# silence-tang/GaussianIP

Measured on AMD Instinct MI355X. Metric: raster_fwd_bwd_mpix_per_s, higher is better.
Workload: dtype f32

## Files before the change

gaussianip_amd/csrc/api.hip:

```cpp
#include <string.h>

#include "gip_internal.h"

static inline size_t align256(size_t x) { return (x + 255) & ~(size_t)255; }

static_assert(offsetof(GipRasterConfig, antialiasing) == 188 && sizeof(GipRasterConfig) == 192, "GipRasterConfig layout");

static bool sh_mfma_path(const GipRasterConfig* c) { return c->sh_coeffs > 0 && c->sh_degree >= 1 && c->V >= 2 && !c->sh_scalar; }

static bool valid_config(const GipRasterConfig* c) {
  if (!c) return false;
  if (c->P < 0 || c->V < 1 || c->V > GIP_MAX_VIEWS || c->H < 1 || c->W < 1) return false;
  if (c->sh_degree < 0 || c->sh_degree > 3) return false;
  if (c->capacity < 1 || c->capacity > 0xfffffff0ull) return false;
  if ((c->H + GIP_TILE - 1) / GIP_TILE > 0xffff || (c->W + GIP_TILE - 1) / GIP_TILE > 0xffff) return false;
  return true;
}

extern "C" int gip_abi_version(void) { return GIP_ABI_VERSION; }

extern "C" const char* gip_status_string(int status) {
  switch (status) {
    case GIP_OK: return "ok";
    case GIP_ERR_BAD_ARGUMENT: return "bad argument (null pointer, or not exactly one of shs/colors_precomp and scales+rotations/cov3D_precomp)";
    case GIP_ERR_BUFFER_TOO_SMALL: return "state or scratch buffer smaller than gip_raster_state_bytes()/gip_raster_scratch_bytes()";
    case GIP_ERR_HIP: return "HIP runtime error";
    case GIP_ERR_UNSUPPORTED: return "unsupported configuration";
    default: return "unknown status";
  }
}

extern "C" int gip_raster_state_layout(const GipRasterConfig* c, GipRasterStateLayout* L) {
  if (!valid_config(c) || !L) return GIP_ERR_BAD_ARGUMENT;
  memset(L, 0, sizeof(*L));
  const size_t P = (size_t)c->P, V = (size_t)c->V;
  L->tiles_x = (uint32_t)((c->W + GIP_TILE - 1) / GIP_TILE);
  L->tiles_y = (uint32_t)((c->H + GIP_TILE - 1) / GIP_TILE);
  L->num_blocks = (uint32_t)((c->P + GIP_BLOCK - 1) / GIP_BLOCK);
  const size_t T = (size_t)L->tiles_x * L->tiles_y, nblk = L->num_blocks;
  size_t off = 0;
  L->header = off;       off = align256(off + sizeof(GipRasterHeader));
  L->tile_count = off;   off = align256(off + V * T * 4);
  L->tile_cursor = off;  off = align256(off + V * T * 4);
  L->tile_count_b = off; off = align256(off + V * T * 4);
  L->tile_start = off;   off = align256(off + (V * T + 1) * 4);
  L->block_sums = off;   off = align256(off + (V * nblk + 1) * 4);
  L->block_offset = off; off = align256(off + (V * nblk + 1) * 4);
  L->records = off;      off = align256(off + V * P * GIP_RECORD_BYTES);
  L->inst_offset = off;  off = align256(off + V * P * 4);
  L->inst_slot = off;    off = align256(off + V * P * GIP_SLOTS * 4);
  L->n_contrib = off;    off = align256(off + V * (size_t)c->H * c->W * 4);
  L->final_T = off;      off = align256(off + V * (size_t)c->H * c->W * 4);
  L->tile_order = off;   off = align256(off + V * T * 4);
  const size_t ckpt_cap = (size_t)c->capacity / GIP_SEGMENT + 1, seg_cap = ckpt_cap + V * T;
  L->seg_start = off;    off = align256(off + (V * T + 1) * 4);
  L->ckpt_start = off;   off = align256(off + (V * T + 1) * 4);
  L->seg_tile = off;     off = align256(off + seg_cap * 4);
  L->checkpoints = off;  off = align256(off + ckpt_cap * GIP_CKPT_FLOATS * 256 * sizeof(float));
  L->keys = off;         off = align256(off + (size_t)c->capacity * 8);
  L->sh_colors = off;    off = align256(off + (sh_mfma_path(c) ? V * P * 4 * sizeof(float) : 0));
  L->total = off;
  return GIP_OK;
}

extern "C" size_t gip_raster_state_bytes(const GipRasterConfig* c) {
  GipRasterStateLayout L;
  if (gip_raster_state_layout(c, &L) != GIP_OK) return 0;
  return L.total;
}

extern "C" size_t gip_raster_scratch_bytes(const GipRasterConfig* c) {
  if (!valid_config(c)) return 0;
  return align256((size_t)c->capacity * GIP_PARTIAL_FLOATS * sizeof(float));
}

static void fill_params(const GipRasterConfig* c, const GipRasterStateLayout& L, GipKernelParams* kp) {
  memset(kp, 0, sizeof(*kp));
  kp->P = c->P; kp->V = c->V; kp->H = c->H; kp->W = c->W;
  kp->tiles_x = (int)L.tiles_x; kp->tiles_y = (int)L.tiles_y; kp->T = kp->tiles_x * kp->tiles_y;
  kp->nblk = (int)L.num_blocks;
  kp->D = c->sh_degree; kp->M = c->sh_coeffs;
  kp->scale_modifier = c->scale_modifier;
  kp->capacity = (uint32_t)c->capacity;
  kp->exact_lists = c->exact_lists ? 1 : 0;
  kp->forward_only = c->forward_only ? 1 : 0;
  kp->sh_mfma = sh_mfma_path(c) ? 1 : 0;
  kp->antialiasing = c->antialiasing ? 1 : 0;
  kp->ckpt_capacity = (uint32_t)(c->capacity / GIP_SEGMENT + 1);
  kp->seg_capacity = kp->ckpt_capacity + (uint32_t)(kp->V * kp->T);
  for (int v = 0; v < c->V; v++) {
    kp->view[v].tanfovx = c->tanfovx[v];
    kp->view[v].tanfovy = c->tanfovy[v];
    kp->view[v].focal_x = c->W / (2.0f * c->tanfovx[v]);
    kp->view[v].focal_y = c->H / (2.0f * c->tanfovy[v]);
  }
}

static GipStatePtrs state_ptrs(void* state, const GipRasterStateLayout& L) {
  char* b = (char*)state;
  GipStatePtrs p;
  p.header = (GipRasterHeader*)(b + L.header);
  p.records = (GipRecord*)(b + L.records);
  p.inst_offset = (uint32_t*)(b + L.inst_offset);
  p.tile_count = (uint32_t*)(b + L.tile_count);
  p.tile_start = (uint32_t*)(b + L.tile_start);
  p.tile_cursor = (uint32_t*)(b + L.tile_cursor);
  p.tile_count_b = (uint32_t*)(b + L.tile_count_b);
  p.inst_slot = (uint32_t*)(b + L.inst_slot);
  p.block_sums = (uint32_t*)(b + L.block_sums);
  p.block_offset = (uint32_t*)(b + L.block_offset);
  p.keys = (unsigned long long*)(b + L.keys);
  p.n_contrib = (uint32_t*)(b + L.n_contrib);
  p.final_T = (float*)(b + L.final_T);
  p.tile_order = (uint32_t*)(b + L.tile_order);
  p.seg_start = (uint32_t*)(b + L.seg_start);
  p.ckpt_start = (uint32_t*)(b + L.ckpt_start);
  p.seg_tile = (uint32_t*)(b + L.seg_tile);
  p.checkpoints = (float*)(b + L.checkpoints);
  p.sh_colors = (float*)(b + L.sh_colors);
  p.host_header = nullptr;
  return p;
}

// ... 42 lines not shown
        float ms = 0.f;
        if (hipEventElapsedTime(&ms, ev[2 * i], ev[2 * i + 1]) != hipSuccess) rc = GIP_ERR_HIP;
        out[i] = ms;
      }
    }
    for (int i = 0; i < created; i++) (void)hipEventDestroy(ev[i]);
    return rc;
  }
};
}

static int forward_impl(const GipRasterConfig* cfg, const GipRasterInputs* in, const GipRasterOutputs* out,
                        void* state, size_t state_bytes, void* stream, float* times) {
  if (!valid_config(cfg)) return cfg && (cfg->V > GIP_MAX_VIEWS || cfg->sh_degree > 3) ? GIP_ERR_UNSUPPORTED : GIP_ERR_BAD_ARGUMENT;
  int rc = check_inputs(cfg, in);
  if (rc != GIP_OK) return rc;
  if (!out || !out->color || !out->radii || !out->depth || !out->alpha || !state) return GIP_ERR_BAD_ARGUMENT;
  GipRasterStateLayout L;
  gip_raster_state_layout(cfg, &L);
  if (state_bytes < L.total) return GIP_ERR_BUFFER_TOO_SMALL;
  GipKernelParams kp;
  fill_params(cfg, L, &kp);
  if (!in->shs) kp.sh_mfma = 0;
  GipStatePtrs st = state_ptrs(state, L);
  st.host_header = out->host_header;
  hipStream_t s = (hipStream_t)stream;
  StageTimer tm(s, times);

  tm.begin(GIP_STAGE_CLEAR);
  HIP_TRY(hipMemsetAsync((char*)state + L.header, 0, L.tile_start - L.header, s));
  tm.end(GIP_STAGE_CLEAR);
  if (cfg->P > 0) {
    tm.begin(GIP_STAGE_PREPROCESS);
    if (kp.sh_mfma) gip_launch_sh_forward_mfma(kp, *in, st.sh_colors, s);
    gip_launch_preprocess(kp, *in, out->radii, st, s);
    tm.end(GIP_STAGE_PREPROCESS);
    LAUNCH_CHECK();
  }
  tm.begin(GIP_STAGE_SCAN);
  gip_launch_scan(kp, st, s);
  tm.end(GIP_STAGE_SCAN);
  LAUNCH_CHECK();
  if (cfg->P > 0) {
    tm.begin(GIP_STAGE_SCATTER);
    gip_launch_scatter(kp, st, s);
    tm.end(GIP_STAGE_SCATTER);
    LAUNCH_CHECK();
// ... 14 lines not shown
  return forward_impl(cfg, in, out, state, state_bytes, stream, nullptr);
}
extern "C" int gip_raster_forward_profiled(const GipRasterConfig* cfg, const GipRasterInputs* in, const GipRasterOutputs* out,
                                           void* state, size_t state_bytes, void* stream, float* times_ms) {
  if (!times_ms) return GIP_ERR_BAD_ARGUMENT;
  return forward_impl(cfg, in, out, state, state_bytes, stream, times_ms);
}

static int backward_impl(const GipRasterConfig* cfg, const GipRasterInputs* in, const GipRasterGradsIn* gin,
                         const void* state, size_t state_bytes, void* scratch, size_t scratch_bytes,
                         const GipRasterGradsOut* gout, void* stream, float* times) {
  if (!valid_config(cfg)) return GIP_ERR_BAD_ARGUMENT;
  int rc = check_inputs(cfg, in);
  if (rc != GIP_OK) return rc;
  if (!gin || !gin->alpha || !gin->color || !gin->depth || !gout || !state || !scratch) return GIP_ERR_BAD_ARGUMENT;
  if (cfg->forward_only) return GIP_ERR_BAD_ARGUMENT;
  GipRasterStateLayout L;
  gip_raster_state_layout(cfg, &L);
  if (state_bytes < L.total || scratch_bytes < gip_raster_scratch_bytes(cfg)) return GIP_ERR_BUFFER_TOO_SMALL;
  if (cfg->P == 0) return GIP_OK;
  GipKernelParams kp;
  fill_params(cfg, L, &kp);
  if (!in->shs) kp.sh_mfma = 0;
  GipStatePtrs st = state_ptrs(const_cast<void*>(state), L);
  hipStream_t s = (hipStream_t)stream;
  StageTimer tm(s, times);
  tm.begin(GIP_STAGE_RENDER_BWD);
  gip_launch_render_backward(kp, in->bg, st, *gin, (float*)scratch, s);
  tm.end(GIP_STAGE_RENDER_BWD);
  LAUNCH_CHECK();
  tm.begin(GIP_STAGE_GATHER_BWD);
  gip_launch_gather_backward(kp, *in, st, (const float*)scratch, *gout, s);
  if (kp.sh_mfma && (gout->dL_dshs || gout->dL_dmeans3D)) gip_launch_sh_backward_mfma(kp, *in, st, st.sh_colors, *gout, s);
  tm.end(GIP_STAGE_GATHER_BWD);
  LAUNCH_CHECK();
  return tm.finish();
}

extern "C" int gip_raster_backward(const GipRasterConfig* cfg, const GipRasterInputs* in, const GipRasterGradsIn* gin,
                                   const void* state, size_t state_bytes, void* scratch, size_t scratch_bytes,
                                   const GipRasterGradsOut* gout, void* stream) {
  return backward_impl(cfg, in, gin, state, state_bytes, scratch, scratch_bytes, gout, stream, nullptr);
}
extern "C" int gip_raster_backward_profiled(const GipRasterConfig* cfg, const GipRasterInputs* in, const GipRasterGradsIn* gin,
                                            const void* state, size_t state_bytes, void* scratch, size_t scratch_bytes,
                                            const GipRasterGradsOut* gout, void* stream, float* times_ms) {
  if (!times_ms) return GIP_ERR_BAD_ARGUMENT;
// ... 18 lines not shown
```

gaussianip_amd/csrc/binning.hip:

```cpp
#include "gip_internal.h"

#define SCAN_THREADS 1024
#define SCAN_WAVES (SCAN_THREADS / 64)
#define SCAN_CHUNK SCAN_THREADS

__device__ __forceinline__ uint32_t nseg_of(uint32_t count) { return (count + GIP_SEGMENT - 1) / GIP_SEGMENT; }

#define ORDER_CLASSES 6
__device__ __forceinline__ int class_of(uint32_t c) {
  return c >= 2048 ? 0 : c >= 1024 ? 1 : c >= 512 ? 2 : c >= 128 ? 3 : c >= 1 ? 4 : 5;
}

__device__ __forceinline__ uint32_t block_excl_scan(uint32_t v, uint32_t* s_w, uint32_t* total) {
  const int lane = threadIdx.x & 63, wave = threadIdx.x >> 6;
  const uint32_t incl = gip_wave_incl_scan_u32(v);
  __syncthreads();
  if (lane == 63) s_w[wave] = incl;
  __syncthreads();
  uint32_t base = 0, tot = 0;
#pragma unroll
  for (int w = 0; w < SCAN_WAVES; w++) { const uint32_t x = s_w[w]; base += w < wave ? x : 0u; tot += x; }
  *total = tot;
  return base + incl - v;
}

__device__ __forceinline__ uint32_t wave_sum_u32(uint32_t v) {
#pragma unroll
  for (int d = 32; d >= 1; d >>= 1) v += (uint32_t)__shfl_xor((int)v, d, 64);
  return v;
}

__global__ void __launch_bounds__(SCAN_THREADS)
gip_scan_kernel(GipKernelParams kp, const uint32_t* __restrict__ tile_count, const uint32_t* __restrict__ tile_count_b,
                uint32_t* __restrict__ tile_start,
                uint32_t* __restrict__ seg_start, uint32_t* __restrict__ ckpt_start,
                const uint32_t* __restrict__ block_sums, uint32_t* __restrict__ block_offset,
                uint32_t* __restrict__ tile_order, GipRasterHeader* __restrict__ header, uint32_t* __restrict__ host_header) {
  __shared__ uint32_t s_w[SCAN_WAVES];
  __shared__ uint32_t s_acc[2][3 + ORDER_CLASSES];
  __shared__ uint32_t s_max;
  __shared__ uint32_t s_cls[ORDER_CLASSES][SCAN_WAVES];
  const int n = kp.V * kp.T;
  const int n_chunks = (n + SCAN_CHUNK - 1) / SCAN_CHUNK;
  const int tid = threadIdx.x, lane = tid & 63, wave = tid >> 6;
  if ((int)blockIdx.x >= n_chunks) {
    const int nb = kp.V * kp.nblk;
    const int c0 = ((int)blockIdx.x - n_chunks) * SCAN_CHUNK;
    uint32_t before = 0;
    for (int i0 = tid; i0 < c0; i0 += 8 * SCAN_THREADS) {
      uint32_t v8[8];
#pragma unroll
      for (int u = 0; u < 8; u++) { const int i = i0 + u * SCAN_THREADS; v8[u] = i < c0 ? block_sums[i] : 0u; }
#pragma unroll
      for (int u = 0; u < 8; u++) before += v8[u];
    }
    before = wave_sum_u32(before);
    if (tid == 0) s_max = 0u;
    __syncthreads();
    if (lane == 0) atomicAdd(&s_max, before);
    __syncthreads();
    const uint32_t base = s_max;
    const int i = c0 + tid;
    const uint32_t v = i < nb ? block_sums[i] : 0u;
    uint32_t total;
    const uint32_t e = block_excl_scan(v, s_w, &total);
    if (i < nb) block_offset[i] = base + e;
    if (c0 + SCAN_CHUNK >= nb && tid == 0) block_offset[nb] = base + total;
    return;
  }
  const int chunk0 = (int)blockIdx.x * SCAN_CHUNK;
  if (tid < 2 * (3 + ORDER_CLASSES)) (&s_acc[0][0])[tid] = 0u;
  if (tid == 0) s_max = 0u;
  __syncthreads();
  uint32_t b_c = 0, b_s = 0, b_k = 0, t_c = 0, t_s = 0, t_k = 0, mx = 0;
  uint32_t b_cls[ORDER_CLASSES], t_cls[ORDER_CLASSES];
#pragma unroll
  for (int c = 0; c < ORDER_CLASSES; c++) { b_cls[c] = 0; t_cls[c] = 0; }
  for (int i0 = wave * 64; i0 < n; i0 += 8 * SCAN_THREADS) {
    uint32_t va[8], vb[8];
#pragma unroll
    for (int u = 0; u < 8; u++) {
      const int i = i0 + u * SCAN_THREADS + lane;
      va[u] = i < n ? tile_count[i] : 0u;
      vb[u] = i < n ? tile_count_b[i] : 0u;
    }
#pragma unroll
    for (int u = 0; u < 8; u++) {
      const int g0 = i0 + u * SCAN_THREADS;
      if (g0 >= n) break;
      const int i = g0 + lane;
      const uint32_t c = va[u] + vb[u], a = nseg_of(c), k = a ? a - 1 : 0;
      const int cls = i < n ? class_of(c) : -1;
      const bool before = g0 < chunk0;
      t_c += c; t_s += a; t_k += k;
      mx = c > mx ? c : mx;
      if (before) { b_c += c; b_s += a; b_k += k; }
#pragma unroll
      for (int q = 0; q < ORDER_CLASSES; q++) {
        const uint32_t m = (uint32_t)__popcll(__ballot(cls == q));
        t_cls[q] += m;
        if (before) b_cls[q] += m;
      }
    }
  }
  b_c = wave_sum_u32(b_c); b_s = wave_sum_u32(b_s); b_k = wave_sum_u32(b_k);
  t_c = wave_sum_u32(t_c); t_s = wave_sum_u32(t_s); t_k = wave_sum_u32(t_k);
  mx = gip_wave_max_u32(mx);
  if (lane == 0) {
    atomicAdd(&s_acc[0][0], b_c); atomicAdd(&s_acc[0][1], b_s); atomicAdd(&s_acc[0][2], b_k);
    atomicAdd(&s_acc[1][0], t_c); atomicAdd(&s_acc[1][1], t_s); atomicAdd(&s_acc[1][2], t_k);
#pragma unroll
    for (int q = 0; q < ORDER_CLASSES; q++) { atomicAdd(&s_acc[0][3 + q], b_cls[q]); atomicAdd(&s_acc[1][3 + q], t_cls[q]); }
    atomicMax(&s_max, mx);
  }
  __syncthreads();
  const int i = chunk0 + tid;
  uint32_t c = 0;
  if (i < n) c = tile_count[i] + tile_count_b[i];
  const uint32_t a = nseg_of(c), k = a ? a - 1 : 0;
  uint32_t tot;
  const uint32_t e_c = block_excl_scan(c, s_w, &tot);
  const uint32_t e_s = block_excl_scan(a, s_w, &tot);
  const uint32_t e_k = block_excl_scan(k, s_w, &tot);
  if (i < n) {
    tile_start[i] = s_acc[0][0] + e_c;
    seg_start[i] = s_acc[0][1] + e_s;
    ckpt_start[i] = s_acc[0][2] + e_k;
  }
  const int cls = i < n ? class_of(c) : -1;
  uint32_t rank = 0;
#pragma unroll
  for (int q = 0; q < ORDER_CLASSES; q++) {
    const unsigned long long m = __ballot(cls == q);
    if (cls == q) rank = (uint32_t)__popcll(m & ((1ull << lane) - 1ull));
    if (lane == 0) s_cls[q][wave] = (uint32_t)__popcll(m);
  }
  __syncthreads();
  if (cls >= 0) {
    uint32_t pos = rank + s_acc[0][3 + cls];
#pragma unroll
    for (int q = 0; q < ORDER_CLASSES; q++) pos += q < cls ? s_acc[1][3 + q] : 0u;
    for (int w = 0; w < wave; w++) pos += s_cls[cls][w];
    tile_order[pos] = (uint32_t)i;
  }
  if (blockIdx.x == 0 && tid == 0) {
    const uint32_t total = s_acc[1][0];
    tile_start[n] = total; seg_start[n] = s_acc[1][1]; ckpt_start[n] = s_acc[1][2];
    const uint32_t n0 = s_acc[1][3], n1 = s_acc[1][4], n2 = s_acc[1][5], n3 = s_acc[1][6], n4 = s_acc[1][7];
    header->class_end[1] = n0;
    header->class_end[2] = n0 + n1;
    header->class_end[0] = n0 + n1 + n2;
    header->class_end[3] = n0 + n1 + n2 + n3 + n4;
    header->abi_version = GIP_ABI_VERSION;
    header->num_rendered = total;
    header->overflow = (total > kp.capacity) ? 1u : 0u;
    header->max_tile_count = s_max;
    header->num_segments = s_acc[1][1];
    header->num_checkpoints = s_acc[1][2];
    if (host_header) {
      host_header[0] = GIP_ABI_VERSION; host_header[1] = total;
      host_header[2] = (total > kp.capacity) ? 1u : 0u; host_header[3] = s_max;
    }
  }
}

void gip_launch_scan(const GipKernelParams& kp, GipStatePtrs st, hipStream_t s) {
  const int n = kp.V * kp.T, nb = kp.V * kp.nblk;
  const int n_chunks = (n + SCAN_CHUNK - 1) / SCAN_CHUNK, b_chunks = nb > 0 ? (nb + SCAN_CHUNK - 1) / SCAN_CHUNK : 1;
  hipLaunchKernelGGL(gip_scan_kernel, dim3(n_chunks + b_chunks), dim3(SCAN_THREADS), 0, s, kp, st.tile_count, st.tile_count_b, st.tile_start,
                     st.seg_start, st.ckpt_start, st.block_sums, st.block_offset, st.tile_order, st.header, st.host_header);
}

__global__ void __launch_bounds__(GIP_BLOCK)
gip_scatter_kernel(GipKernelParams kp, const GipRecord* __restrict__ records, const uint32_t* __restrict__ tile_start,
                   const uint32_t* __restrict__ tile_count, uint32_t* __restrict__ tile_cursor,
                   const uint32_t* __restrict__ inst_slot, const uint32_t* __restrict__ block_offset,
                   uint32_t* __restrict__ inst_offset, unsigned long long* __restrict__ keys) {
  const int v = blockIdx.y;
  const int idx = blockIdx.x * GIP_BLOCK + threadIdx.x;
  uint32_t tiles = 0, rmin = 0, rmax = 0, dbits = 0, tmask = 0;
  if (idx < kp.P) {
    const uint4* rp = reinterpret_cast<const uint4*>(records + (size_t)v * kp.P + idx);
    const uint4 q0 = rp[0], q1 = rp[1], q3 = rp[3];
    dbits = q0.z; tiles = q1.w; rmin = q3.x; rmax = q3.y; tmask = q3.w;
  }
  __shared__ uint32_t s_wave[4];
  const int lane = threadIdx.x & 63, wave = threadIdx.x >> 6;
  uint32_t incl = gip_wave_incl_scan_u32(tiles);
  if (lane == 63) s_wave[wave] = incl;
  __syncthreads();
  uint32_t base = block_offset[(size_t)v * kp.nblk + blockIdx.x];
  for (int w = 0; w < wave; w++) base += s_wave[w];
  if (idx < kp.P) inst_offset[(size_t)v * kp.P + idx] = base + incl - tiles;
// ... 389 lines not shown
```

gaussianip_amd/csrc/gip_internal.h:

```cpp
#pragma once
#include <hip/hip_runtime.h>
#include <stdint.h>

#include "../../include/gip_raster.h"

#define GIP_BLOCK 256
#define GIP_WAVE 64
#define GIP_NEAR 0.2f
#define GIP_ALPHA_MIN (1.0f / 255.0f)
#define GIP_ALPHA_MAX 0.99f
#define GIP_T_MIN 0.0001f

struct __attribute__((aligned(16))) GipRecord {
  float x, y, depth, opacity;
  float ca, cb, cc; uint32_t tiles;
  float r, g, b; int32_t radius;
  uint32_t rmin, rmax, clamped, tmask;
};

#define GIP_MASK_TILES 32
__host__ __device__ inline bool gip_rect_has(uint32_t tmask, int area, int k) { return area > GIP_MASK_TILES || ((tmask >> k) & 1u); }
__host__ __device__ inline int gip_rect_rank(uint32_t tmask, int area, int k) {
  return area > GIP_MASK_TILES ? k : __builtin_popcount(tmask & ((1u << k) - 1u));
}

static_assert(sizeof(GipRecord) == GIP_RECORD_BYTES, "record size");

struct GipViewConst {
  float tanfovx, tanfovy, focal_x, focal_y;
};

struct GipKernelParams {
  int P, V, H, W;
  int tiles_x, tiles_y, T;
  int nblk;
  int D, M;
  float scale_modifier;
  uint32_t capacity;
  uint32_t seg_capacity;
  uint32_t ckpt_capacity;
  int exact_lists;
  int forward_only;
  int sh_mfma;
  int antialiasing;
  GipViewConst view[GIP_MAX_VIEWS];
};

struct GipStatePtrs {
  GipRasterHeader* header;
  GipRecord* records;
  uint32_t* inst_offset;
  uint32_t* tile_count;
  uint32_t* tile_start;
  uint32_t* tile_cursor;
  uint32_t* tile_count_b;
  uint32_t* inst_slot;
  uint32_t* block_sums;
  uint32_t* block_offset;
  unsigned long long* keys;
  uint32_t* n_contrib;
  float* final_T;
  uint32_t* tile_order;
  uint32_t* seg_start;
  uint32_t* ckpt_start;
  uint32_t* seg_tile;
  float* checkpoints;
  uint32_t* host_header;
  float* sh_colors;
};

void gip_launch_preprocess(const GipKernelParams& kp, const GipRasterInputs& in, int32_t* radii, GipStatePtrs st, hipStream_t s);
void gip_launch_scan(const GipKernelParams& kp, GipStatePtrs st, hipStream_t s);
void gip_launch_scatter(const GipKernelParams& kp, GipStatePtrs st, hipStream_t s);
void gip_launch_tile_sort(const GipKernelParams& kp, GipStatePtrs st, hipStream_t s);
void gip_launch_render_forward(const GipKernelParams& kp, const float* bg, GipStatePtrs st, float* color, float* depth, float* alpha, hipStream_t s);
void gip_launch_render_backward(const GipKernelParams& kp, const float* bg, GipStatePtrs st, const GipRasterGradsIn& gin, float* partial, hipStream_t s);
void gip_launch_gather_backward(const GipKernelParams& kp, const GipRasterInputs& in, GipStatePtrs st, const float* partial, const GipRasterGradsOut& gout, hipStream_t s);
void gip_launch_sh_forward_mfma(const GipKernelParams& kp, const GipRasterInputs& in, float* sh_colors, hipStream_t s);
void gip_launch_sh_backward_mfma(const GipKernelParams& kp, const GipRasterInputs& in, GipStatePtrs st, const float* sh_gcol, const GipRasterGradsOut& gout, hipStream_t s);
void gip_launch_mark_visible(int P, const float* means3D, const float* view, uint8_t* present, hipStream_t s);

#ifdef __HIPCC__
__device__ __forceinline__ uint32_t gip_wave_incl_scan_u32(uint32_t v) {
  const int lane = threadIdx.x & 63;
#pragma unroll
  for (int d = 1; d < 64; d <<= 1) {
    uint32_t o = __shfl_up(v, d, 64);
    if (lane >= d) v += o;
  }
  return v;
}
// ... 13 lines not shown
```

gaussianip_amd/csrc/render_forward.hip:

```cpp
#include <stdlib.h>

#include "gip_internal.h"

#ifndef FWD_PAIRS
#define FWD_PAIRS 4
#endif
#define FWD_THREADS 512
typedef float v2f __attribute__((ext_vector_type(2)));
typedef float v4f __attribute__((ext_vector_type(4)));

__device__ __forceinline__ float xchg32(float x, int hh) {
  float a = x, b = x;
  asm volatile("s_nop 1\n\tv_permlane32_swap_b32 %0, %1\n\ts_nop 1" : "+v"(a), "+v"(b));
  return hh ? a : b;
}

__device__ __forceinline__ void both32(float x, float& lo, float& hi) {
  lo = x; hi = x;
  asm volatile("s_nop 1\n\tv_permlane32_swap_b32 %0, %1\n\ts_nop 1" : "+v"(lo), "+v"(hi));
}

__device__ __forceinline__ int ffs_clear(unsigned long long& m) {
  int j;
  asm volatile("s_ff1_i32_b64 %0, %1\n\ts_bitset0_b64 %1, %0" : "=&s"(j), "+s"(m));
  return j;
}

__global__ void __launch_bounds__(FWD_THREADS)
gip_render_forward_kernel(GipKernelParams kp, const uint32_t* __restrict__ tile_order,
                          const uint32_t* __restrict__ tile_start, const unsigned long long* __restrict__ keys,
                          const GipRecord* __restrict__ records, const float* __restrict__ bg,
                          float* __restrict__ out_color, float* __restrict__ out_depth, float* __restrict__ out_alpha,
                          uint32_t* __restrict__ n_contrib, float* __restrict__ final_T, const uint32_t* __restrict__ ckpt_start,
                          float* __restrict__ checkpoints) {
  const uint32_t pos = blockIdx.x;
  const uint32_t vt = tile_order[pos];
  const uint32_t v = vt / kp.T, tile = vt - v * kp.T;
  const uint32_t tx = tile % kp.tiles_x, ty = tile / kp.tiles_x;
  const int lane = threadIdx.x & 63, wave = threadIdx.x >> 6;
  const int hh = lane >> 5, pl = lane & 31;
  const int lx = ((wave & 1) << 3) | (pl & 7), ly = ((wave >> 1) << 2) | (pl >> 3);
  const int px = tx * GIP_TILE + lx, py = ty * GIP_TILE + ly;
  const bool inside = px < kp.W && py < kp.H;
  const v2f pxy = {(float)px, (float)py};
  const float tile_x0 = (float)(tx * GIP_TILE), tile_y0 = (float)(ty * GIP_TILE);
  const int cpix = ((((ly >> 3) << 1) | (lx >> 3)) << 6) | ((ly & 7) << 3) | (lx & 7);

  const uint32_t start = tile_start[vt];
  uint32_t end = tile_start[vt + 1];
  if (end > kp.capacity) end = kp.capacity;
  if (end < start) end = start;
  const GipRecord* recs = records + (size_t)v * kp.P;

  constexpr int FWD_SLOTS = (FWD_THREADS / 64) * 65;
  __shared__ v2f s_xy[FWD_SLOTS];
  __shared__ v4f s_con[FWD_SLOTS];
  __shared__ v4f s_col[FWD_SLOTS];
  __shared__ uint32_t s_mask[FWD_THREADS];
  if (threadIdx.x < FWD_THREADS / 64) {
    s_xy[threadIdx.x * 65] = (v2f){0.f, 0.f};
    s_con[threadIdx.x * 65] = (v4f){0.f, 0.f, 0.f, 0.f};
    s_col[threadIdx.x * 65] = (v4f){0.f, 0.f, 0.f, 0.f};
  }
  const int sidx = threadIdx.x + (threadIdx.x >> 6) + 1;

  bool done = !inside;
  float T = 1.0f, Wt = 0.f;
  v2f CG = {0.f, 0.f}, BD = {0.f, 0.f};
  uint32_t last_contributor = 0;
  int last_off = -1;

  uint32_t g_next = 0xffffffffu, g_next2 = 0xffffffffu;
  float4 r0 = make_float4(0.f, 0.f, 0.f, 0.f), r1 = r0, r2 = r0;
  if (start + threadIdx.x < end) g_next = (uint32_t)keys[start + threadIdx.x];
  if (start + FWD_THREADS + threadIdx.x < end) g_next2 = (uint32_t)keys[start + FWD_THREADS + threadIdx.x];
  if (g_next != 0xffffffffu) {
    const float4* rp = reinterpret_cast<const float4*>(recs + g_next);
    r0 = rp[0]; r1 = rp[1]; r2 = rp[2];
  }

  for (uint32_t base = start; base < end; base += FWD_THREADS) {
    if (__syncthreads_count(done) == FWD_THREADS) break;
    const uint32_t k = base + threadIdx.x;
    if (k < end) {
      const float4 q0 = r0, q1 = r1, q2 = r2;
      s_xy[sidx] = (v2f){q0.x, q0.y};
      s_con[sidx] = (v4f){q1.x * -0.72134752044448170f, q1.z * -0.72134752044448170f, q1.y * -1.4426950408889634f, q0.w};
      s_col[sidx] = (v4f){q2.x, q2.y, q2.z, q0.z};
      uint32_t mask = 0xff;
      const float t2 = 2.0f * __logf(255.0f * q0.w) + 0.02f;
      const float det = q1.x * q1.z - q1.y * q1.y;
      if (t2 <= 0.f) {
        mask = 0;
      } else if (det > 0.f) {
        const float inv = t2 / det;
        const float hx = sqrtf(inv * q1.z) * 1.01f + 0.05f, hy = sqrtf(inv * q1.x) * 1.01f + 0.05f;
        const float rx = q0.x - tile_x0, ry = q0.y - tile_y0;
        const uint32_t cols = (rx - hx <= 7.f ? 1u : 0u) | (rx + hx >= 8.f ? 2u : 0u);
        const float ylo = ry - hy, yhi = ry + hy;
        const float hd = 0.5f * (q1.x - q1.z);
        const float lmax = 0.5f * (q1.x + q1.z) + sqrtf(__builtin_fmaf(hd, hd, q1.y * q1.y));
        const float rad = sqrtf(inv * lmax) * 1.01f + 0.05f;
        const float rad2 = rad * rad;
        const float ex0 = fmaxf(fmaxf(-rx, rx - 7.f), 0.f), ex1 = fmaxf(fmaxf(8.f - rx, rx - 15.f), 0.f);
        const float ex0s = ex0 * ex0, ex1s = ex1 * ex1;
        mask = 0;
#pragma unroll
        for (int band = 0; band < 4; band++) {
          const float ey = fmaxf(fmaxf((float)(4 * band) - ry, ry - (float)(4 * band + 3)), 0.f);
          const float eys = ey * ey;
          const uint32_t near = (ex0s + eys <= rad2 ? 1u : 0u) | (ex1s + eys <= rad2 ? 2u : 0u);
          if (ylo <= (float)(4 * band + 3) && yhi >= (float)(4 * band)) mask |= (cols & near) << (2 * band);
        }
      }
      s_mask[threadIdx.x] = mask;
    }
    g_next = g_next2;
    g_next2 = (k + 2 * FWD_THREADS < end) ? (uint32_t)keys[k + 2 * FWD_THREADS] : 0xffffffffu;
    if (g_next != 0xffffffffu) {
      const float4* rp = reinterpret_cast<const float4*>(recs + g_next);
      r0 = rp[0]; r1 = rp[1]; r2 = rp[2];
    }
    __syncthreads();
    const int cnt = min((uint32_t)FWD_THREADS, end - base);
    if (!__all(done)) {
      for (int c0 = 0; c0 < cnt; c0 += 64) {
        const uint32_t rel = (base - start) + c0;
        if (rel != 0 && (rel % GIP_SEGMENT) == 0) {
          const float s0 = CG.x + xchg32(CG.x, hh), s1 = CG.y + xchg32(CG.y, hh), s2 = BD.x + xchg32(BD.x, hh), sd = BD.y + xchg32(BD.y, hh);
          const uint32_t slot = ckpt_start[vt] + rel / GIP_SEGMENT - 1;
          if (slot < kp.ckpt_capacity && hh == 0 && !kp.forward_only && !done) {
            float* cp = checkpoints + (size_t)slot * (GIP_CKPT_FLOATS * GIP_BLOCK) + cpix;
            cp[0] = T; cp[GIP_BLOCK] = s0; cp[2 * GIP_BLOCK] = s1; cp[3 * GIP_BLOCK] = s2; cp[4 * GIP_BLOCK] = sd;
          }
        }
        const int e = c0 + lane;
        const uint32_t mk = e < cnt ? s_mask[e] : 0u;
        unsigned long long m = __ballot((mk >> wave) & 1u);
        const int cbase16 = ((c0 >> 6) * 65 + 1) << 4;
        bool wave_done = false;
        while (m) {
          int ja[FWD_PAIRS];
          float al[FWD_PAIRS];
          v4f cc[FWD_PAIRS];
#pragma unroll
          for (int u = 0; u < FWD_PAIRS; u++) {
            const int j1 = ffs_clear(m), j2 = ffs_clear(m);
            const int a1 = cbase16 + (j1 << 4), a2 = cbase16 + (j2 << 4);
            ja[u] = hh ? a2 : a1;
            const v2f d = *(const v2f*)((const char*)s_xy + (ja[u] >> 1)) - pxy;
            const v4f co = *(const v4f*)((const char*)s_con + ja[u]);
            cc[u] = *(const v4f*)((const char*)s_col + ja[u]);
            const v2f t = co.xy * d;
            const float power = __builtin_fmaf(d.x, __builtin_fmaf(co.z, d.y, t.x), t.y * d.y);
            const float a = fminf(GIP_ALPHA_MAX, co.w * __builtin_amdgcn_exp2f(power));
            al[u] = (power <= 0.0f && a >= GIP_ALPHA_MIN) ? a : 0.f;
          }
          const unsigned long long done_before = __ballot(done);
#pragma unroll
          for (int u = 0; u < FWD_PAIRS; u++) {
            float a_e, a_o;
            both32(al[u], a_e, a_o);
            a_e = done ? 0.f : a_e;
            const float t1 = __builtin_fmaf(-a_e, T, T);
            const bool stop1 = t1 < GIP_T_MIN;
            const float T1 = stop1 ? T : t1;
            a_o = (done || stop1) ? 0.f : a_o;
            const float t2 = __builtin_fmaf(-a_o, T1, T1);
            const bool stop2 = t2 < GIP_T_MIN;
            const float w_e = stop1 ? 0.f : a_e * T, w_o = stop2 ? 0.f : a_o * T1;
            const float w = hh ? w_o : w_e;
            CG = __builtin_elementwise_fma(cc[u].xy, (v2f){w, w}, CG);
            BD = __builtin_elementwise_fma(cc[u].zw, (v2f){w, w}, BD);
            Wt += w;
            last_off = w > 0.f ? ja[u] : last_off;
            T = stop2 ? T1 : t2;
            done = done || stop1 || stop2;
          }
          if (__ballot(done) != done_before) {
            if (__all(done)) { wave_done = true; break; }
          }
        }
        if (wave_done) break;
      }
    }
    if (last_off >= 0) {
      const uint32_t slot = (uint32_t)last_off >> 4;
      last_contributor = (base - start) + slot - slot / 65u;
      last_off = -1;
    }
  }

  float C0 = CG.x, C1 = CG.y, C2 = BD.x, Dp = BD.y;
  C0 += xchg32(C0, hh); C1 += xchg32(C1, hh); C2 += xchg32(C2, hh); Wt += xchg32(Wt, hh); Dp += xchg32(Dp, hh);
  const uint32_t lc_other = __float_as_uint(xchg32(__uint_as_float(last_contributor), hh));
  last_contributor = max(last_contributor, lc_other);
  if (inside && hh == 0) {
    const size_t HW = (size_t)kp.H * kp.W;
    const size_t pix = (size_t)py * kp.W + px;
    float* oc = out_color + (size_t)v * 3 * HW;
    oc[pix] = C0 + T * bg[0];
    oc[HW + pix] = C1 + T * bg[1];
    oc[2 * HW + pix] = C2 + T * bg[2];
    out_depth[(size_t)v * HW + pix] = Dp;
    out_alpha[(size_t)v * HW + pix] = Wt;
    if (!kp.forward_only) {
      n_contrib[(size_t)v * HW + pix] = last_contributor;
      final_T[(size_t)v * HW + pix] = T;
    }
  }
}


void gip_launch_render_forward(const GipKernelParams& kp, const float* bg, GipStatePtrs st, float* color, float* depth,
                               float* alpha, hipStream_t s) {
  hipLaunchKernelGGL(gip_render_forward_kernel, dim3(kp.V * kp.T), dim3(FWD_THREADS), 0, s, kp, st.tile_order,
                     st.tile_start, st.keys, st.records, bg, color, depth, alpha, st.n_contrib, st.final_T, st.ckpt_start,
                     st.checkpoints);
}
```

Measured before the change: 8504.

## Split long tile lists across blocks in forward render and compose partial results

Tiles whose Gaussian lists hold at least FWD_LONG entries are split into FWD_CHUNK-sized chunks. Each chunk is rendered by its own block and writes partial transmittance and colour rows. A new compose kernel then merges the chunks in order, rescales the stored checkpoints, and replays a chunk exactly when the accumulated transmittance falls near the stop threshold. The goal is to remove the load imbalance where a few very long tiles dominate forward render time. The cost is extra launches, extra state memory, more scan work, and duplicated work on chunks that an early-terminating earlier chunk would have skipped.

```diff
diff --git a/gaussianip_amd/csrc/api.hip b/gaussianip_amd/csrc/api.hip
--- a/gaussianip_amd/csrc/api.hip
+++ b/gaussianip_amd/csrc/api.hip
@@ -15,6 +15,19 @@
   if (c->capacity < 1 || c->capacity > 0xfffffff0ull) return false;
   if ((c->H + GIP_TILE - 1) / GIP_TILE > 0xffff || (c->W + GIP_TILE - 1) / GIP_TILE > 0xffff) return false;
   return true;
+}
+
+struct FwdLongLayout { size_t row_start, done, xitems, rows, end; uint32_t xcap, row_cap; };
+static FwdLongLayout fwd_long_layout(const GipRasterConfig* c, size_t off, size_t VT) {
+  FwdLongLayout F;
+  F.xcap = (uint32_t)(c->capacity / FWD_CHUNK + 1);
+  F.row_cap = (uint32_t)(2 * (c->capacity / FWD_CHUNK) + 2);
+  F.row_start = off; off = align256(off + VT * 4);
+  F.done = off;      off = align256(off + VT * 4);
+  F.xitems = off;    off = align256(off + (size_t)F.xcap * 8);
+  F.rows = off;      off = align256(off + (size_t)F.row_cap * FWD_ROW_FLOATS * 256 * sizeof(float));
+  F.end = off;
+  return F;
 }
 
 extern "C" int gip_abi_version(void) { return GIP_ABI_VERSION; }
@@ -58,6 +71,7 @@
   L->seg_tile = off;     off = align256(off + seg_cap * 4);
   L->checkpoints = off;  off = align256(off + ckpt_cap * GIP_CKPT_FLOATS * 256 * sizeof(float));
   L->keys = off;         off = align256(off + (size_t)c->capacity * 8);
+  off = fwd_long_layout(c, off, V * T).end;
   L->sh_colors = off;    off = align256(off + (sh_mfma_path(c) ? V * P * 4 * sizeof(float) : 0));
   L->total = off;
   return GIP_OK;
@@ -88,6 +102,8 @@
   kp->antialiasing = c->antialiasing ? 1 : 0;
   kp->ckpt_capacity = (uint32_t)(c->capacity / GIP_SEGMENT + 1);
   kp->seg_capacity = kp->ckpt_capacity + (uint32_t)(kp->V * kp->T);
+  kp->fwd_xcap = (uint32_t)(c->capacity / FWD_CHUNK + 1);
+  kp->fwd_row_cap = (uint32_t)(2 * (c->capacity / FWD_CHUNK) + 2);
   for (int v = 0; v < c->V; v++) {
     kp->view[v].tanfovx = c->tanfovx[v];
     kp->view[v].tanfovy = c->tanfovy[v];
@@ -96,9 +112,14 @@
   }
 }
 
-static GipStatePtrs state_ptrs(void* state, const GipRasterStateLayout& L) {
+static GipStatePtrs state_ptrs(const GipRasterConfig* c, void* state, const GipRasterStateLayout& L) {
   char* b = (char*)state;
   GipStatePtrs p;
+  const FwdLongLayout F = fwd_long_layout(c, align256(L.keys + (size_t)c->capacity * 8), (size_t)c->V * L.tiles_x * L.tiles_y);
+  p.fwd_row_start = (uint32_t*)(b + F.row_start);
+  p.fwd_done = (uint32_t*)(b + F.done);
+  p.fwd_xitems = (uint32_t*)(b + F.xitems);
+  p.fwd_rows = (float*)(b + F.rows);
   p.header = (GipRasterHeader*)(b + L.header);
   p.records = (GipRecord*)(b + L.records);
   p.inst_offset = (uint32_t*)(b + L.inst_offset);
@@ -187,7 +208,7 @@
   GipKernelParams kp;
   fill_params(cfg, L, &kp);
   if (!in->shs) kp.sh_mfma = 0;
-  GipStatePtrs st = state_ptrs(state, L);
+  GipStatePtrs st = state_ptrs(cfg, state, L);
   st.host_header = out->host_header;
   hipStream_t s = (hipStream_t)stream;
   StageTimer tm(s, times);
@@ -248,7 +269,7 @@
   GipKernelParams kp;
   fill_params(cfg, L, &kp);
   if (!in->shs) kp.sh_mfma = 0;
-  GipStatePtrs st = state_ptrs(const_cast<void*>(state), L);
+  GipStatePtrs st = state_ptrs(cfg, const_cast<void*>(state), L);
   hipStream_t s = (hipStream_t)stream;
   StageTimer tm(s, times);
   tm.begin(GIP_STAGE_RENDER_BWD);
diff --git a/gaussianip_amd/csrc/binning.hip b/gaussianip_amd/csrc/binning.hip
--- a/gaussianip_amd/csrc/binning.hip
+++ b/gaussianip_amd/csrc/binning.hip
@@ -35,9 +35,10 @@
                 uint32_t* __restrict__ tile_start,
                 uint32_t* __restrict__ seg_start, uint32_t* __restrict__ ckpt_start,
                 const uint32_t* __restrict__ block_sums, uint32_t* __restrict__ block_offset,
-                uint32_t* __restrict__ tile_order, GipRasterHeader* __restrict__ header, uint32_t* __restrict__ host_header) {
+                uint32_t* __restrict__ tile_order, GipRasterHeader* __restrict__ header, uint32_t* __restrict__ host_header,
+                uint32_t* __restrict__ fwd_row_start, uint32_t* __restrict__ fwd_done, uint32_t* __restrict__ fwd_xitems) {
   __shared__ uint32_t s_w[SCAN_WAVES];
-  __shared__ uint32_t s_acc[2][3 + ORDER_CLASSES];
+  __shared__ uint32_t s_acc[2][5 + ORDER_CLASSES];
   __shared__ uint32_t s_max;
   __shared__ uint32_t s_cls[ORDER_CLASSES][SCAN_WAVES];
   const int n = kp.V * kp.T;
@@ -69,10 +70,11 @@
     return;
   }
   const int chunk0 = (int)blockIdx.x * SCAN_CHUNK;
-  if (tid < 2 * (3 + ORDER_CLASSES)) (&s_acc[0][0])[tid] = 0u;
+  if (tid < 2 * (5 + ORDER_CLASSES)) (&s_acc[0][0])[tid] = 0u;
   if (tid == 0) s_max = 0u;
   __syncthreads();
   uint32_t b_c = 0, b_s = 0, b_k = 0, t_c = 0, t_s = 0, t_k = 0, mx = 0;
+  uint32_t b_r = 0, b_x = 0, t_x = 0;
   uint32_t b_cls[ORDER_CLASSES], t_cls[ORDER_CLASSES];
 #pragma unroll
   for (int c = 0; c < ORDER_CLASSES; c++) { b_cls[c] = 0; t_cls[c] = 0; }
@@ -92,9 +94,10 @@
       const uint32_t c = va[u] + vb[u], a = nseg_of(c), k = a ? a - 1 : 0;
       const int cls = i < n ? class_of(c) : -1;
       const bool before = g0 < chunk0;
-      t_c += c; t_s += a; t_k += k;
+      const uint32_t fr = gip_fwd_chunks(c), fx = fr ? fr - 1 : 0;
+      t_c += c; t_s += a; t_k += k; t_x += fx;
       mx = c > mx ? c : mx;
-      if (before) { b_c += c; b_s += a; b_k += k; }
+      if (before) { b_c += c; b_s += a; b_k += k; b_r += fr; b_x += fx; }
 #pragma unroll
       for (int q = 0; q < ORDER_CLASSES; q++) {
         const uint32_t m = (uint32_t)__popcll(__ballot(cls == q));
@@ -105,8 +108,10 @@
   }
   b_c = wave_sum_u32(b_c); b_s = wave_sum_u32(b_s); b_k = wave_sum_u32(b_k);
   t_c = wave_sum_u32(t_c); t_s = wave_sum_u32(t_s); t_k = wave_sum_u32(t_k);
+  b_r = wave_sum_u32(b_r); b_x = wave_sum_u32(b_x); t_x = wave_sum_u32(t_x);
   mx = gip_wave_max_u32(mx);
   if (lane == 0) {
+    atomicAdd(&s_acc[0][3 + ORDER_CLASSES], b_r); atomicAdd(&s_acc[0][4 + ORDER_CLASSES], b_x); atomicAdd(&s_acc[1][4 + ORDER_CLASSES], t_x);
     atomicAdd(&s_acc[0][0], b_c); atomicAdd(&s_acc[0][1], b_s); atomicAdd(&s_acc[0][2], b_k);
     atomicAdd(&s_acc[1][0], t_c); atomicAdd(&s_acc[1][1], t_s); atomicAdd(&s_acc[1][2], t_k);
 #pragma unroll
@@ -122,10 +127,18 @@
   const uint32_t e_c = block_excl_scan(c, s_w, &tot);
   const uint32_t e_s = block_excl_scan(a, s_w, &tot);
   const uint32_t e_k = block_excl_scan(k, s_w, &tot);
+  const uint32_t fr = gip_fwd_chunks(c), fx = fr ? fr - 1 : 0;
+  const uint32_t e_r = block_excl_scan(fr, s_w, &tot);
+  const uint32_t e_x = block_excl_scan(fx, s_w, &tot);
   if (i < n) {
     tile_start[i] = s_acc[0][0] + e_c;
     seg_start[i] = s_acc[0][1] + e_s;
     ckpt_start[i] = s_acc[0][2] + e_k;
+    fwd_row_start[i] = s_acc[0][3 + ORDER_CLASSES] + e_r;
+    fwd_done[i] = 0u;
+    const uint32_t x0 = s_acc[0][4 + ORDER_CLASSES] + e_x;
+    for (uint32_t q = 0; q < fx; q++)
+      if (x0 + q < kp.fwd_xcap) { fwd_xitems[2 * (x0 + q)] = (uint32_t)i; fwd_xitems[2 * (x0 + q) + 1] = q + 1; }
   }
   const int cls = i < n ? class_of(c) : -1;
   uint32_t rank = 0;
@@ -157,6 +170,8 @@
     header->max_tile_count = s_max;
     header->num_segments = s_acc[1][1];
     header->num_checkpoints = s_acc[1][2];
+    header->reserved[0] = s_acc[1][4 + ORDER_CLASSES];
+    header->reserved[1] = FWD_LONG == 1024 ? n0 + n1 : n0;
     if (host_header) {
       host_header[0] = GIP_ABI_VERSION; host_header[1] = total;
       host_header[2] = (total > kp.capacity) ? 1u : 0u; host_header[3] = s_max;
@@ -168,7 +183,8 @@
   const int n = kp.V * kp.T, nb = kp.V * kp.nblk;
   const int n_chunks = (n + SCAN_CHUNK - 1) / SCAN_CHUNK, b_chunks = nb > 0 ? (nb + SCAN_CHUNK - 1) / SCAN_CHUNK : 1;
   hipLaunchKernelGGL(gip_scan_kernel, dim3(n_chunks + b_chunks), dim3(SCAN_THREADS), 0, s, kp, st.tile_count, st.tile_count_b, st.tile_start,
-                     st.seg_start, st.ckpt_start, st.block_sums, st.block_offset, st.tile_order, st.header, st.host_header);
+                     st.seg_start, st.ckpt_start, st.block_sums, st.block_offset, st.tile_order, st.header, st.host_header,
+                     st.fwd_row_start, st.fwd_done, st.fwd_xitems);
 }
 
 __global__ void __launch_bounds__(GIP_BLOCK)
diff --git a/gaussianip_amd/csrc/gip_internal.h b/gaussianip_amd/csrc/gip_internal.h
--- a/gaussianip_amd/csrc/gip_internal.h
+++ b/gaussianip_amd/csrc/gip_internal.h
@@ -10,6 +10,19 @@
 #define GIP_ALPHA_MIN (1.0f / 255.0f)
 #define GIP_ALPHA_MAX 0.99f
 #define GIP_T_MIN 0.0001f
+
+#ifndef FWD_LONG
+#define FWD_LONG 1024
+#endif
+#ifndef FWD_CHUNK
+#define FWD_CHUNK 1024
+#endif
+#define FWD_ROW_FLOATS 8
+#define FWD_NEAR_STOP 0.0002f
+static_assert(FWD_LONG == 1024 || FWD_LONG == 2048, "FWD_LONG must be a size-class bound of the scan");
+static_assert(FWD_LONG % 512 == 0 && FWD_LONG % GIP_SEGMENT == 0 && FWD_CHUNK % 512 == 0 && FWD_CHUNK % GIP_SEGMENT == 0 && FWD_CHUNK <= FWD_LONG,
+              "FWD_LONG / FWD_CHUNK: multiples of the 512-entry batch and of GIP_SEGMENT");
+__host__ __device__ inline uint32_t gip_fwd_chunks(uint32_t count) { return count >= FWD_LONG ? (count + FWD_CHUNK - 1) / FWD_CHUNK : 0u; }
 
 struct __attribute__((aligned(16))) GipRecord {
   float x, y, depth, opacity;
@@ -43,6 +56,8 @@
   int forward_only;
   int sh_mfma;
   int antialiasing;
+  uint32_t fwd_xcap;
+  uint32_t fwd_row_cap;
   GipViewConst view[GIP_MAX_VIEWS];
 };
 
@@ -67,6 +82,10 @@
   float* checkpoints;
   uint32_t* host_header;
   float* sh_colors;
+  uint32_t* fwd_row_start;
+  uint32_t* fwd_done;
+  uint32_t* fwd_xitems;
+  float* fwd_rows;
 };
 
 void gip_launch_preprocess(const GipKernelParams& kp, const GipRasterInputs& in, int32_t* radii, GipStatePtrs st, hipStream_t s);
diff --git a/gaussianip_amd/csrc/render_forward.hip b/gaussianip_amd/csrc/render_forward.hip
--- a/gaussianip_amd/csrc/render_forward.hip
+++ b/gaussianip_amd/csrc/render_forward.hip
@@ -32,9 +32,24 @@
                           const GipRecord* __restrict__ records, const float* __restrict__ bg,
                           float* __restrict__ out_color, float* __restrict__ out_depth, float* __restrict__ out_alpha,
                           uint32_t* __restrict__ n_contrib, float* __restrict__ final_T, const uint32_t* __restrict__ ckpt_start,
-                          float* __restrict__ checkpoints) {
-  const uint32_t pos = blockIdx.x;
-  const uint32_t vt = tile_order[pos];
+                          float* __restrict__ checkpoints, const GipRasterHeader* __restrict__ header,
+                          const uint32_t* __restrict__ fwd_row_start, uint32_t* fwd_done, const uint32_t* __restrict__ fwd_xitems,
+                          float* __restrict__ fwd_rows) {
+  uint32_t pos = blockIdx.x, chunk = 0;
+  const uint32_t n_long = header->reserved[1], n_extra = min(header->reserved[0], kp.fwd_xcap);
+  const bool lng = pos < n_long + n_extra;
+  uint32_t vt;
+  if (pos < n_long) {
+    vt = tile_order[pos];
+  } else if (lng) {
+    vt = fwd_xitems[2 * (pos - n_long)];
+    chunk = fwd_xitems[2 * (pos - n_long) + 1];
+  } else {
+    pos -= n_extra;
+    if (pos >= (uint32_t)(kp.V * kp.T)) return;
+    vt = tile_order[pos];
+  }
+  const float t_min = chunk ? -1.0f : GIP_T_MIN;
   const uint32_t v = vt / kp.T, tile = vt - v * kp.T;
   const uint32_t tx = tile % kp.tiles_x, ty = tile / kp.tiles_x;
   const int lane = threadIdx.x & 63, wave = threadIdx.x >> 6;
@@ -51,6 +66,15 @@
   if (end > kp.capacity) end = kp.capacity;
   if (end < start) end = start;
   const GipRecord* recs = records + (size_t)v * kp.P;
+  const uint32_t cstart = start + chunk * FWD_CHUNK;
+  const uint32_t cend = lng ? min(end, cstart + FWD_CHUNK) : end;
+  if (chunk) {
+    if (cstart >= end) return;
+    __shared__ uint32_t s_fin;
+    if (threadIdx.x == 0) s_fin = __hip_atomic_load(&fwd_done[vt], __ATOMIC_RELAXED, __HIP_MEMORY_SCOPE_AGENT);
+    __syncthreads();
+    if (s_fin) return;
+  }
 
   constexpr int FWD_SLOTS = (FWD_THREADS / 64) * 65;
   __shared__ v2f s_xy[FWD_SLOTS];
@@ -72,17 +96,17 @@
 
   uint32_t g_next = 0xffffffffu, g_next2 = 0xffffffffu;
   float4 r0 = make_float4(0.f, 0.f, 0.f, 0.f), r1 = r0, r2 = r0;
-  if (start + threadIdx.x < end) g_next = (uint32_t)keys[start + threadIdx.x];
-  if (start + FWD_THREADS + threadIdx.x < end) g_next2 = (uint32_t)keys[start + FWD_THREADS + threadIdx.x];
+  if (cstart + threadIdx.x < cend) g_next = (uint32_t)keys[cstart + threadIdx.x];
+  if (cstart + FWD_THREADS + threadIdx.x < cend) g_next2 = (uint32_t)keys[cstart + FWD_THREADS + threadIdx.x];
   if (g_next != 0xffffffffu) {
     const float4* rp = reinterpret_cast<const float4*>(recs + g_next);
     r0 = rp[0]; r1 = rp[1]; r2 = rp[2];
   }
 
-  for (uint32_t base = start; base < end; base += FWD_THREADS) {
+  for (uint32_t base = cstart; base < cend; base += FWD_THREADS) {
     if (__syncthreads_count(done) == FWD_THREADS) break;
     const uint32_t k = base + threadIdx.x;
-    if (k < end) {
+    if (k < cend) {
       const float4 q0 = r0, q1 = r1, q2 = r2;
       s_xy[sidx] = (v2f){q0.x, q0.y};
       s_con[sidx] = (v4f){q1.x * -0.72134752044448170f, q1.z * -0.72134752044448170f, q1.y * -1.4426950408889634f, q0.w};
@@ -116,13 +140,13 @@
       s_mask[threadIdx.x] = mask;
     }
     g_next = g_next2;
-    g_next2 = (k + 2 * FWD_THREADS < end) ? (uint32_t)keys[k + 2 * FWD_THREADS] : 0xffffffffu;
+    g_next2 = (k + 2 * FWD_THREADS < cend) ? (uint32_t)keys[k + 2 * FWD_THREADS] : 0xffffffffu;
     if (g_next != 0xffffffffu) {
       const float4* rp = reinterpret_cast<const float4*>(recs + g_next);
       r0 = rp[0]; r1 = rp[1]; r2 = rp[2];
     }
     __syncthreads();
-    const int cnt = min((uint32_t)FWD_THREADS, end - base);
+    const int cnt = min((uint32_t)FWD_THREADS, cend - base);
     if (!__all(done)) {
       for (int c0 = 0; c0 < cnt; c0 += 64) {
         const uint32_t rel = (base - start) + c0;
@@ -163,11 +187,11 @@
             both32(al[u], a_e, a_o);
             a_e = done ? 0.f : a_e;
             const float t1 = __builtin_fmaf(-a_e, T, T);
-            const bool stop1 = t1 < GIP_T_MIN;
+            const bool stop1 = t1 < t_min;
             const float T1 = stop1 ? T : t1;
             a_o = (done || stop1) ? 0.f : a_o;
             const float t2 = __builtin_fmaf(-a_o, T1, T1);
-            const bool stop2 = t2 < GIP_T_MIN;
+            const bool stop2 = t2 < t_min;
             const float w_e = stop1 ? 0.f : a_e * T, w_o = stop2 ? 0.f : a_o * T1;
             const float w = hh ? w_o : w_e;
             CG = __builtin_elementwise_fma(cc[u].xy, (v2f){w, w}, CG);
@@ -195,6 +219,19 @@
   C0 += xchg32(C0, hh); C1 += xchg32(C1, hh); C2 += xchg32(C2, hh); Wt += xchg32(Wt, hh); Dp += xchg32(Dp, hh);
   const uint32_t lc_other = __float_as_uint(xchg32(__uint_as_float(last_contributor), hh));
   last_contributor = max(last_contributor, lc_other);
+  if (lng) {
+    const uint32_t row = fwd_row_start[vt] + chunk;
+    if (hh == 0 && row < kp.fwd_row_cap) {
+      float* rp = fwd_rows + (size_t)row * (FWD_ROW_FLOATS * GIP_BLOCK) + cpix;
+      rp[0] = T; rp[GIP_BLOCK] = C0; rp[2 * GIP_BLOCK] = C1; rp[3 * GIP_BLOCK] = C2; rp[4 * GIP_BLOCK] = Dp; rp[5 * GIP_BLOCK] = Wt;
+      rp[6 * GIP_BLOCK] = __uint_as_float(last_contributor); rp[7 * GIP_BLOCK] = __uint_as_float(done ? 1u : 0u);
+    }
+    if (chunk == 0) {
+      const bool all_done = __syncthreads_count(done) == FWD_THREADS;
+      if (all_done && threadIdx.x == 0) __hip_atomic_store(&fwd_done[vt], 1u, __ATOMIC_RELAXED, __HIP_MEMORY_SCOPE_AGENT);
+    }
+    return;
+  }
   if (inside && hh == 0) {
     const size_t HW = (size_t)kp.H * kp.W;
     const size_t pix = (size_t)py * kp.W + px;
@@ -212,9 +249,142 @@
 }
 
 
+struct FwdPix { float T, C0, C1, C2, D, W; uint32_t last; bool done; };
+__device__ __forceinline__ void fwd_entry(FwdPix& p, v2f xy, v4f co, v4f cc, v2f pxy, uint32_t index1) {
+  const v2f d = xy - pxy;
+  const v2f t = co.xy * d;
+  const float power = __builtin_fmaf(d.x, __builtin_fmaf(co.z, d.y, t.x), t.y * d.y);
+  float a = fminf(GIP_ALPHA_MAX, co.w * __builtin_amdgcn_exp2f(power));
+  a = (power <= 0.0f && a >= GIP_ALPHA_MIN && !p.done) ? a : 0.f;
+  const float t1 = __builtin_fmaf(-a, p.T, p.T);
+  const bool stop = t1 < GIP_T_MIN;
+  const float w = stop ? 0.f : a * p.T;
+  p.C0 = __builtin_fmaf(cc.x, w, p.C0); p.C1 = __builtin_fmaf(cc.y, w, p.C1); p.C2 = __builtin_fmaf(cc.z, w, p.C2);
+  p.D = __builtin_fmaf(cc.w, w, p.D); p.W += w;
+  p.last = w > 0.f ? index1 : p.last;
+  p.T = stop ? p.T : t1;
+  p.done = p.done || stop;
+}
+
+#define CMP_THREADS GIP_BLOCK
+__global__ void __launch_bounds__(CMP_THREADS)
+gip_forward_compose_kernel(GipKernelParams kp, const GipRasterHeader* __restrict__ header, const uint32_t* __restrict__ tile_order,
+                           const uint32_t* __restrict__ tile_start, const unsigned long long* __restrict__ keys,
+                           const GipRecord* __restrict__ records, const float* __restrict__ bg, float* __restrict__ out_color,
+                           float* __restrict__ out_depth, float* __restrict__ out_alpha, uint32_t* __restrict__ n_contrib,
+                           float* __restrict__ final_T, const uint32_t* __restrict__ ckpt_start, float* checkpoints,
+                           const uint32_t* __restrict__ fwd_row_start, const float* __restrict__ fwd_rows) {
+  __shared__ v2f s_xy[CMP_THREADS];
+  __shared__ v4f s_con[CMP_THREADS];
+  __shared__ v4f s_col[CMP_THREADS];
+  const uint32_t n_long = header->reserved[1];
+  const int tid = threadIdx.x, lane = tid & 63, wbase = tid & ~63;
+  const int lx = (((tid >> 6) & 1) << 3) | (tid & 7), ly = ((tid >> 7) << 3) | ((tid >> 3) & 7);
+  for (uint32_t pos = blockIdx.x; pos < n_long; pos += gridDim.x) {
+    const uint32_t vt = tile_order[pos];
+    const uint32_t v = vt / kp.T, tile = vt - v * kp.T;
+    const uint32_t tx = tile % kp.tiles_x, ty = tile / kp.tiles_x;
+    const int px = tx * GIP_TILE + lx, py = ty * GIP_TILE + ly;
+    const bool inside = px < kp.W && py < kp.H;
+    const v2f pxy = {(float)px, (float)py};
+    const uint32_t start = tile_start[vt];
+    uint32_t end = tile_start[vt + 1];
+    if (end > kp.capacity) end = kp.capacity;
+    if (end < start) end = start;
+    const uint32_t n = end - start;
+    const uint32_t row0 = fwd_row_start[vt], ck0 = ckpt_start[vt];
+    uint32_t nc = (n + FWD_CHUNK - 1) / FWD_CHUNK;
+    if (row0 >= kp.fwd_row_cap) continue;
+    if (row0 + nc > kp.fwd_row_cap) nc = kp.fwd_row_cap - row0;
+    const GipRecord* recs = records + (size_t)v * kp.P;
+    const float* r0 = fwd_rows + (size_t)row0 * (FWD_ROW_FLOATS * GIP_BLOCK) + tid;
+    FwdPix p;
+    p.T = r0[0]; p.C0 = r0[GIP_BLOCK]; p.C1 = r0[2 * GIP_BLOCK]; p.C2 = r0[3 * GIP_BLOCK]; p.D = r0[4 * GIP_BLOCK];
+    p.W = r0[5 * GIP_BLOCK]; p.last = __float_as_uint(r0[6 * GIP_BLOCK]);
+    p.done = !inside || __float_as_uint(r0[7 * GIP_BLOCK]) != 0u;
+    for (uint32_t c = 1; c < nc; c++) {
+      const float* rc = r0 + (size_t)c * (FWD_ROW_FLOATS * GIP_BLOCK);
+      const uint32_t cs = c * FWD_CHUNK, ce = min(n, cs + FWD_CHUNK);
+      float Tl = 1.f, L0 = 0.f, L1 = 0.f, L2 = 0.f, Ld = 0.f, Lw = 0.f;
+      uint32_t Ll = 0;
+      if (!p.done) {
+        Tl = rc[0]; L0 = rc[GIP_BLOCK]; L1 = rc[2 * GIP_BLOCK]; L2 = rc[3 * GIP_BLOCK]; Ld = rc[4 * GIP_BLOCK];
+        Lw = rc[5 * GIP_BLOCK]; Ll = __float_as_uint(rc[6 * GIP_BLOCK]);
+      }
+      const bool replay = !p.done && !(p.T * Tl >= FWD_NEAR_STOP);
+      if (!p.done && !replay) {
+        if (!kp.forward_only) {
+#pragma unroll 4
+          for (uint32_t rel = cs; rel < ce; rel += GIP_SEGMENT) {
+            const uint32_t slot = ck0 + rel / GIP_SEGMENT - 1;
+            if (slot < kp.ckpt_capacity) {
+              float* cp = checkpoints + (size_t)slot * (GIP_CKPT_FLOATS * GIP_BLOCK) + tid;
+              const float kT = cp[0], k0 = cp[GIP_BLOCK], k1 = cp[2 * GIP_BLOCK], k2 = cp[3 * GIP_BLOCK], kd = cp[4 * GIP_BLOCK];
+              cp[0] = p.T * kT; cp[GIP_BLOCK] = __builtin_fmaf(p.T, k0, p.C0); cp[2 * GIP_BLOCK] = __builtin_fmaf(p.T, k1, p.C1);
+              cp[3 * GIP_BLOCK] = __builtin_fmaf(p.T, k2, p.C2); cp[4 * GIP_BLOCK] = __builtin_fmaf(p.T, kd, p.D);
+            }
+          }
+        }
+        p.C0 = __builtin_fmaf(p.T, L0, p.C0); p.C1 = __builtin_fmaf(p.T, L1, p.C1); p.C2 = __builtin_fmaf(p.T, L2, p.C2);
+        p.D = __builtin_fmaf(p.T, Ld, p.D); p.W = __builtin_fmaf(p.T, Lw, p.W);
+        p.last = Ll ? Ll : p.last;
+        p.T *= Tl;
+      }
+      if (__any(replay)) {
+        for (uint32_t e0 = cs; e0 < ce; e0 += 64) {
+          if (!__any(replay && !p.done)) break;
+          const uint32_t e = e0 + lane;
+          if (e < ce) {
+            const uint32_t g = (uint32_t)keys[start + e];
+            const float4* rp = reinterpret_cast<const float4*>(recs + g);
+            const float4 q0 = rp[0], q1 = rp[1], q2 = rp[2];
+            s_xy[tid] = (v2f){q0.x, q0.y};
+            s_con[tid] = (v4f){q1.x * -0.72134752044448170f, q1.z * -0.72134752044448170f, q1.y * -1.4426950408889634f, q0.w};
+            s_col[tid] = (v4f){q2.x, q2.y, q2.z, q0.z};
+          }
+          __builtin_amdgcn_fence(__ATOMIC_RELEASE, "wavefront");
+          __builtin_amdgcn_wave_barrier();
+          __builtin_amdgcn_fence(__ATOMIC_ACQUIRE, "wavefront");
+          const uint32_t slot = ck0 + e0 / GIP_SEGMENT - 1;
+          if ((e0 % GIP_SEGMENT) == 0 && !kp.forward_only && slot < kp.ckpt_capacity && replay && !p.done) {
+            float* cp = checkpoints + (size_t)slot * (GIP_CKPT_FLOATS * GIP_BLOCK) + tid;
+            cp[0] = p.T; cp[GIP_BLOCK] = p.C0; cp[2 * GIP_BLOCK] = p.C1; cp[3 * GIP_BLOCK] = p.C2; cp[4 * GIP_BLOCK] = p.D;
+          }
+          const int cnt = (int)min(64u, ce - e0);
+          if (replay) {
+            for (int j = 0; j < cnt; j++)
+              fwd_entry(p, s_xy[wbase + j], s_con[wbase + j], s_col[wbase + j], pxy, e0 + j + 1);
+          }
+          __builtin_amdgcn_fence(__ATOMIC_RELEASE, "wavefront");
+          __builtin_amdgcn_wave_barrier();
+          __builtin_amdgcn_fence(__ATOMIC_ACQUIRE, "wavefront");
+        }
+      }
+    }
+    if (inside) {
+      const size_t HW = (size_t)kp.H * kp.W;
+      const size_t pix = (size_t)py * kp.W + px;
+      float* oc = out_color + (size_t)v * 3 * HW;
+      oc[pix] = p.C0 + p.T * bg[0];
+      oc[HW + pix] = p.C1 + p.T * bg[1];
+      oc[2 * HW + pix] = p.C2 + p.T * bg[2];
+      out_depth[(size_t)v * HW + pix] = p.D;
+      out_alpha[(size_t)v * HW + pix] = p.W;
+      if (!kp.forward_only) {
+        n_contrib[(size_t)v * HW + pix] = p.last;
+        final_T[(size_t)v * HW + pix] = p.T;
+      }
+    }
+  }
+}
+
 void gip_launch_render_forward(const GipKernelParams& kp, const float* bg, GipStatePtrs st, float* color, float* depth,
                                float* alpha, hipStream_t s) {
-  hipLaunchKernelGGL(gip_render_forward_kernel, dim3(kp.V * kp.T), dim3(FWD_THREADS), 0, s, kp, st.tile_order,
+  hipLaunchKernelGGL(gip_render_forward_kernel, dim3(kp.V * kp.T + kp.fwd_xcap), dim3(FWD_THREADS), 0, s, kp, st.tile_order,
                      st.tile_start, st.keys, st.records, bg, color, depth, alpha, st.n_contrib, st.final_T, st.ckpt_start,
-                     st.checkpoints);
-}
+                     st.checkpoints, st.header, st.fwd_row_start, st.fwd_done, st.fwd_xitems, st.fwd_rows);
+  const int tiles = kp.V * kp.T;
+  hipLaunchKernelGGL(gip_forward_compose_kernel, dim3(tiles < 1024 ? tiles : 1024), dim3(CMP_THREADS), 0, s, kp, st.header,
+                     st.tile_order, st.tile_start, st.keys, st.records, bg, color, depth, alpha, st.n_contrib, st.final_T,
+                     st.ckpt_start, st.checkpoints, st.fwd_row_start, st.fwd_rows);
+}
```

Result: slower. 5414 (-36.3%).
